# eigenkernel/eigenkernel

Hardware: AMD Instinct MI355X
Metric: eigenpairs/s (full spectrum) + achieved fp64 TFLOP/s vs roofline, N=16384 GEP (higher is better)
Workload: dtype f64

## Files before the change

### eigenkernel_amd/csrc/ek_chol.hip

```cpp
#include "ek_common.h"
#include "ek_block64.h"

#include <cstdlib>
#include <vector>

namespace ek {
namespace {

constexpr int NB = kDiagNB;
constexpr size_t kDiagLds = 2 * b64::IMG * sizeof(double);

__global__ __launch_bounds__(256) void potrf_diag_kernel(int nb, double *B, int ldb, double *inv, int *info,
                                                         int info_base) {
  using namespace b64;
  extern __shared__ double smem[];
  double *sP = smem, *sQ = smem + IMG;
  __shared__ double s_scr[kScratch];
  const int t = threadIdx.x, lane = t & 63, wave = t >> 6, l15 = lane & 15, l4 = lane >> 4;
  auto upper = [&](int gr, int gc) -> double {
    if (gc < nb) return B[(size_t)gc + (size_t)gr * ldb];
    return (gr == gc) ? 1.0 : 0.0;
  };
  auto fail_exit = [&](int j) {
    if (t == 0) atomicCAS(info, 0, info_base + j + 1);
// ... 198 lines not shown
  static bool attr_set = false;
  if (attr_set) return;
  (void)hipFuncSetAttribute((const void *)potrf_diag_kernel, hipFuncAttributeMaxDynamicSharedMemorySize, kDiagLds);
  (void)hipFuncSetAttribute((const void *)trtri_diag_kernel,
                            hipFuncAttributeMaxDynamicSharedMemorySize, (NB * NB + NB) * sizeof(double));
  attr_set = true;
}

void potrf_lower(hipStream_t s, int n, double *B, int ldb, double *invdiag, int *d_info,
                 double *work) {
  set_attrs();
  if (n <= 0) return;
  potrf_rec(s, n, B, ldb, 0, invdiag, d_info, work);
}

void trtri256_blocks(hipStream_t s, int n, const double *L, int ldl, const double *invdiag, double *inv256, double *scratch) {
  const int nb2 = n / (2 * NB);
  if (nb2 <= 0) return;
  GemmDesc g{};
  g.M = NB; g.N = NB; g.K = NB; g.transA = false; g.transB = false; g.alpha = 1.0; g.beta = 0.0; g.batch = nb2; g.lower_only = false;
  g.A = L + NB; g.lda = ldl; g.strideA = (long long)2 * NB * ((long long)ldl + 1);
  g.B = invdiag; g.ldb = NB; g.strideB = (long long)2 * NB * NB;
  g.C = scratch; g.ldc = NB; g.strideC = (long long)NB * NB;
  gemm(s, g);
  g.alpha = -1.0;
  g.A = invdiag + (size_t)NB * NB; g.lda = NB; g.strideA = (long long)2 * NB * NB;
  g.B = scratch; g.ldb = NB; g.strideB = (long long)NB * NB;
  g.C = inv256 + NB; g.ldc = 2 * NB; g.strideC = (long long)4 * NB * NB;
  gemm(s, g);
  hipLaunchKernelGGL(inv256_assemble_kernel, dim3(nb2), dim3(256), 0, s, invdiag, inv256);
}
void trsm_register_inv256(const double *invdiag, const double *inv256, int n) {
  g_inv256.base128 = inv256 ? invdiag : nullptr; g_inv256.inv256 = inv256; g_inv256.nblk256 = inv256 ? n / (2 * NB) : 0;
// ... 123 lines not shown
int sygst_set_direct(int order) {
  const int before = g_sygst_direct;
  g_sygst_direct = order <= 0 ? kSygstDirect : (order < 2 * NB ? 2 * NB : order);
  return before;
}
void sygst_scratch_need(int n, size_t need[2]) {
  if (n <= sygst_direct()) return;
  const size_t n1 = (size_t)split_t(n), n2 = (size_t)n - n1;
  const size_t t1 = n1 * n1 + n1 * n2, t2 = (n1 > n2 ? n1 : n2) * (size_t)n;
  if (t1 > need[0]) need[0] = t1;
  if (t2 > need[1]) need[1] = t2;
  sygst_scratch_need((int)n1, need);
  sygst_scratch_need((int)n2, need);
}

static void sygst_rec(hipStream_t s, int n, double *A, int lda, const double *L, int ldl,
                      const double *invdiag, double *work, double *scratch) {
  if (n <= 0) return;
  if (n <= sygst_direct()) {
    symmetrize_lower(s, n, A, lda);
    trsm_lln(s, n, n, L, ldl, invdiag, A, lda, work);
    trsm_rlt_lower(s, n, L, ldl, invdiag, A, lda, work);
    return;
  }
  const int n1 = split_t(n), n2 = n - n1;
  double *A21 = A + n1, *A22 = A + (size_t)n1 + (size_t)n1 * lda;
  const double *L21 = L + n1, *L22 = L + (size_t)n1 + (size_t)n1 * ldl;
  const double *inv2 = invdiag + (size_t)(n1 / NB) * NB * NB;
  sygst_rec(s, n1, A, lda, L, ldl, invdiag, work, scratch);
  trsm_rlt(s, n2, n1, L, ldl, invdiag, A21, lda, work);
  double *C11 = scratch, *M = scratch + (size_t)n1 * n1;
  hipLaunchKernelGGL(full_from_lower_kernel, grid_mn(n1, n1), dim3(256), 0, s, n1, A, lda, C11, n1);
  gemm(s, false, false, n2, n1, n1, 1.0, L21, ldl, C11, n1, 0.0, M, n2);
  hipLaunchKernelGGL(axpy_matrix_kernel, grid_mn(n2, n1), dim3(256), 0, s, n2, n1, -0.5, M, n2, A21, lda);
  if (n2 <= n1) {
    double *P = C11;
    gemm(s, false, true, n2, n2, n1, 1.0, A21, lda, L21, ldl, 0.0, P, n2);
    hipLaunchKernelGGL(syr2k_fold_kernel, dim3(ceil_div(n2, 32), ceil_div(n2, 32)), dim3(256), 0, s, n2, P, n2, A22, lda);
  } else {
    gemm(s, false, true, n2, n2, n1, -1.0, A21, lda, L21, ldl, 1.0, A22, lda, true);
    gemm(s, false, true, n2, n2, n1, -1.0, L21, ldl, A21, lda, 1.0, A22, lda, true);
  }
  hipLaunchKernelGGL(axpy_matrix_kernel, grid_mn(n2, n1), dim3(256), 0, s, n2, n1, -0.5, M, n2, A21, lda);
  trsm_lln(s, n2, n1, L22, ldl, inv2, A21, lda, work);
  sygst_rec(s, n2, A22, lda, L22, ldl, inv2, work, scratch);
}

void sygst_lower(hipStream_t s, int n, double *A, int lda, const double *L, int ldl,
                 const double *invdiag, double *work, double *scratch) {
  if (n <= 0) return;
  sygst_rec(s, n, A, lda, L, ldl, invdiag, work, scratch);
}


__global__ __launch_bounds__(256) void trmm_diag_kernel(int n, int ldd, const double *__restrict__ L, int ldl,
                                                        double *__restrict__ diag) {
  const int b = blockIdx.x, off = b * ldd;
  const int nb = n - off < ldd ? n - off : ldd;
  double *D = diag + (size_t)b * ldd * ldd;
  const int per = ldd * ldd / gridDim.y;
  for (int idx = blockIdx.y * per + threadIdx.x; idx < (blockIdx.y + 1) * per; idx += 256) {
    const int i = idx % ldd, j = idx / ldd;
    D[idx] = (i >= j && i < nb) ? L[(size_t)(off + i) + (size_t)(off + j) * ldl] : 0.0;
  }
}
int trmm_block_ld(int n) { return n > kDiagNB ? 2 * NB : NB; }
// ... 288 lines not shown
      if (e0) { g_pprof.mark(s); g_pprof.kind.push_back(1); }
      if (has_next) issue_strip(s, k + 1, cur ^ 1);
      waited = true;
    }
  }
  for (int m = 0; m < nmem; ++m)
    hipLaunchKernelGGL(info_to_double_kernel, dim3(ceil_div(NRB, 256)), dim3(256), 0, s, NRB, infos[m], infod[m]);
  x.allreduce(s, nmem, infod, (size_t)NRB, x.user);
  for (int m = 0; m < nmem; ++m)
    hipLaunchKernelGGL(first_info_kernel, dim3(1), dim3(64), 0, s, NRB, infod[m], mem[m].d_info);
}

size_t potrf_rl_work_bytes(int n, int ld) { return PotrfDistLayout(n, ld, 1).total; }

void potrf_lower_rl(hipStream_t s, hipStream_t s2, int n, double *B, int ldb, double *invdiag, int *d_info,
                    void *work) {
  set_attrs();
  if (n <= 0) return;
  const PotrfDistLayout Ly(n, ldb, 1);
  const int NRB = Ly.NRB;
  char *w = (char *)work;
  double *ppan = (double *)(w + Ly.off_pbuf);
  int *infos = (int *)(w + Ly.off_infos);
  double *infod = (double *)(w + Ly.off_infod);
  long long *offs = (long long *)(w + Ly.off_offs);
  int *dims = (int *)(w + Ly.off_dims);
  static hipEvent_t evU[2], evP[2], evFork;
  static bool ev_ready = false;
  if (!ev_ready) {
    for (int i = 0; i < 2; ++i) {
      (void)hipEventCreateWithFlags(&evU[i], hipEventDisableTiming);
      (void)hipEventCreateWithFlags(&evP[i], hipEventDisableTiming);
    }
    (void)hipEventCreateWithFlags(&evFork, hipEventDisableTiming);
    ev_ready = true;
  }
  (void)hipMemsetAsync(infos, 0, (size_t)NRB * sizeof(int), s);
  hipLaunchKernelGGL(potrf_table_kernel, dim3(NRB), dim3(round_up(Ly.maxb, 64)), 0, s, n, ldb, 1, 0, NRB, Ly.maxb,
                     offs, dims);
  auto factor_panel = [&](hipStream_t st, int k) {
    const int off = k * NB, nbk = (n - off < NB) ? n - off : NB, mrows = n - off - nbk;
    double *Bd = B + (size_t)off + (size_t)off * ldb;
    double *inv = invdiag + (size_t)k * NB * NB;
    hipLaunchKernelGGL(potrf_diag_kernel, dim3(1), dim3(256), kDiagLds, st, nbk, Bd,
                       ldb, inv, infos + k, off);
    if (mrows > 0) {
      gemm(st, false, true, mrows, nbk, nbk, 1.0, Bd + nbk, ldb, inv, NB, 0.0, ppan, mrows);
      copy_matrix(st, mrows, nbk, ppan, mrows, Bd + nbk, ldb);
    }
// ... 5 lines not shown
    for (int k = k0; k < k1; ++k) {
      factor_panel(st, k);
      const int cnt = k1 - 1 - k;
      if (cnt > 0) {
        const int nbk = (n - k * NB < NB) ? n - k * NB : NB;
        GemmDesc g{};
        g.N = NB; g.K = nbk; g.transA = false; g.transB = true; g.alpha = -1.0; g.beta = 1.0;
        g.A = B; g.lda = ldb; g.B = B; g.ldb = ldb; g.C = B; g.ldc = ldb; g.lower_only = true;
        g.even_offs = true;
        g.M = n - (k + 1) * NB; g.batch = cnt;
        g.d_offs = offs + (size_t)k * Ly.maxb * 3; g.d_dims = dims + (size_t)k * Ly.maxb * 3;
        gemm(st, g);
      }
    }
  };
  (void)hipEventRecord(evFork, s);
  (void)hipStreamWaitEvent(s2, evFork, 0);
  factor_outer(s2, 0);
  (void)hipEventRecord(evP[0], s2);
  for (int o = 0; o + 1 < NOB; ++o) {
    const int c0 = o * ob * NB, c1 = (o + 1) * ob * NB, kw = c1 - c0;
    const int m2 = n - c1;
    const int wnext = (m2 < ob * NB) ? m2 : ob * NB;
    (void)hipStreamWaitEvent(s, evP[o & 1], 0);
    const double *P = B + (size_t)c1 + (size_t)c0 * ldb;
    double *C = B + (size_t)c1 + (size_t)c1 * ldb;
    gemm(s, false, true, m2, wnext, kw, -1.0, P, ldb, P, ldb, 1.0, C, ldb, true);
    (void)hipEventRecord(evU[(o + 1) & 1], s);
    if (m2 > wnext)
      gemm(s, false, true, m2 - wnext, m2 - wnext, kw, -1.0, P + wnext, ldb, P + wnext, ldb, 1.0,
           C + (size_t)wnext + (size_t)wnext * ldb, ldb, true);
    (void)hipStreamWaitEvent(s2, evU[(o + 1) & 1], 0);
    factor_outer(s2, o + 1);
    (void)hipEventRecord(evP[(o + 1) & 1], s2);
  }
  (void)hipStreamWaitEvent(s, evP[(NOB - 1) & 1], 0);
  hipLaunchKernelGGL(info_to_double_kernel, dim3(ceil_div(NRB, 256)), dim3(256), 0, s, NRB, infos, infod);
  hipLaunchKernelGGL(first_info_kernel, dim3(1), dim3(64), 0, s, NRB, infod, d_info);
}

size_t sygst_dist_scratch_doubles(int n, int ld, int nranks) {
  const int NRB = ceil_div(n > 0 ? n : 1, NB);
  return (size_t)ld * NB * ceil_div(NRB, nranks > 0 ? nranks : 1);
}

void sygst_lower_dist(hipStream_t s, int n, int nmem, const SygstMember *mem, const SytrdExchange &x) {
  if (n <= 0 || nmem <= 0 || nmem > kMaxTeam) return;
  const int P = x.nranks;
  const int NRB = ceil_div(n, NB);
  const int wblk = ceil_div(NRB, P) * NB;
  size_t offs[kMaxTeam], counts[kMaxTeam];
  for (int r = 0; r < P; ++r) {
    long long c0 = (long long)r * wblk, c1 = c0 + wblk;
// ... 34 lines not shown
```

### eigenkernel_amd/csrc/ek_common.h

```cpp
#pragma once
#include <hip/hip_runtime.h>
#include <cstddef>
#include <cstdint>
#include <cstdio>

#define EK_HIP_CHECK(expr)                                                              \
  do {                                                                                  \
    hipError_t _e = (expr);                                                             \
    if (_e != hipSuccess) {                                                             \
      fprintf(stderr, "[ek_hip] %s failed at %s:%d: %s\n", #expr, __FILE__, __LINE__,   \
              hipGetErrorString(_e));                                                   \
      return -1000 - (int)_e;                                                           \
    }                                                                                   \
  } while (0)

namespace ek {

constexpr int kWave = 64;

inline int ceil_div(int a, int b) { return (a + b - 1) / b; }
inline int round_up(int a, int b) { return ceil_div(a, b) * b; }

struct GemmDesc {
  int M, N, K;
// ... 59 lines not shown
constexpr int kDiagNB = 128;
void potrf_lower(hipStream_t s, int n, double *B, int ldb, double *invdiag, int *d_info,
                 double *work );
void trtri_diag_blocks(hipStream_t s, int n, const double *L, int ldl, double *invdiag);
void trsm_rlt(hipStream_t s, int m, int n, const double *L, int ldl, const double *invdiag,
              double *X, int ldx, double *work);
void trsm_lln(hipStream_t s, int n, int m, const double *L, int ldl, const double *invdiag,
              double *X, int ldx, double *work);
void trsm_llt(hipStream_t s, int n, int m, const double *L, int ldl, const double *invdiag,
              double *X, int ldx, double *work);
inline size_t sygst_scratch_doubles(int n) {
  const size_t h = (size_t)(n / 2 + 128);
  const size_t a = 2 * h * h, b = 2 * 128 * 128;
  return a > b ? a : b;
}
void trtri256_blocks(hipStream_t s, int n, const double *L, int ldl, const double *invdiag, double *inv256, double *scratch);
void trsm_register_inv256(const double *invdiag, const double *inv256, int n);
void sygst_lower(hipStream_t s, int n, double *A, int lda, const double *L, int ldl,
                 const double *invdiag, double *work, double *scratch);
int sygst_set_direct(int order);
void sygst_scratch_need(int n, size_t need[2]);
int trmm_block_ld(int n);
size_t trmm_diag_doubles(int n);
void trmm_diag_blocks(hipStream_t s, int n, const double *L, int ldl, double *diag);
void trmm_rln(hipStream_t s, int m, int n, const double *L, int ldl, const double *diag, int ldd,
              double *X, int ldx, double *work);
void trmm_llt(hipStream_t s, int n, int m, const double *L, int ldl, const double *diag, int ldd,
              double *X, int ldx, double *work);
void trmm_lln(hipStream_t s, int n, int m, const double *L, int ldl, const double *diag, int ldd,
              double *X, int ldx, double *work);
void sygst2_lower(hipStream_t s, int n, double *A, int lda, const double *L, int ldl, const double *diag,
                  double *work, double *scratch);
struct SygstMember {
  double *A; int lda; const double *L; int ldl; const double *invdiag;
  double *work;
  double *scratch;
  int rank;
};
size_t potrf_rl_work_bytes(int n, int ld);
void potrf_lower_rl(hipStream_t s, hipStream_t s2, int n, double *B, int ldb, double *invdiag, int *d_info,
                    void *work);
struct SytrdExchange;
struct PotrfMember { double *B; int ldb; double *invdiag; int *d_info; void *work; int rank; };
size_t potrf_dist_work_bytes(int n, int ld, int nranks);
void potrf_lower_dist(hipStream_t s, hipStream_t s2, int n, int nmem, const PotrfMember *mem, const SytrdExchange &x);
void potrf_dist_set_lookahead(int on);
void potrf_dist_profile(bool on);
void potrf_dist_profile_collect(double *seconds, int P);
size_t sygst_dist_scratch_doubles(int n, int ld, int nranks);
void sygst_lower_dist(hipStream_t s, int n, int nmem, const SygstMember *mem, const SytrdExchange &x);

struct SytrdWork;
size_t sytrd_work_bytes(int n);
void sytrd_lower(hipStream_t s, int n, double *A, int lda, double *d, double *e, double *tau,
                 double *V, int ldv, void *work);

// ... 105 lines not shown
```

### eigenkernel_amd/csrc/ek_debug.hip

```cpp
#include "ek_api_internal.h"

using namespace ek;
using namespace ek::api;

extern "C" {

int ek_hip_potrf_team(int n, double *B_loc, const int desc_B[9], int nteam, long long *mismatch) {
  if (n < 0) return -1;
  if (!B_loc && n > 0) return -2;
  int rc = check_desc(desc_B, 3, n, n); if (rc) return rc;
  if (nteam < 0 || nteam > kMaxTeam) return -4;
  rc = ensure_init(); if (rc) return rc;
  if (mismatch) *mismatch = 0;
  if (n == 0) return 0;
  std::lock_guard<std::mutex> lk(g_mu);
  if (nteam == 0 && !g_comm.on) return -4;
  hipStream_t s = g_ctx.stream;
  const int ld = pad_ld(n), nblk = ceil_div(n, kDiagNB);
  const int nmem = nteam > 0 ? nteam : 1, P = nteam > 0 ? nteam : g_comm.nranks;
  const size_t wb = potrf_dist_work_bytes(n, ld, P);
  const size_t per = al((size_t)ld * ld * 8) + al((size_t)nblk * kDiagNB * kDiagNB * 8) + al(wb) + 256;
  void *ws;
  rc = workspace(per * nmem + 256, &ws);
  if (rc) return rc;
// ... 206 lines not shown
  return sy2sb_on_host_arrays(n, A, lda, V, ldv, tau, 0, flag);
}

int ek_hip_debug_sy2sb_stage(int n, double *A, int lda, double *V, int ldv, double *tau, int poison, int *flag) {
  if (n < 1) return -1;
  if (!A) return -2;
  if (lda < n) return -3;
  if (!V) return -4;
  if (ldv < n) return -5;
  if (!tau) return -6;
  if (!flag) return -8;
  return sy2sb_on_host_arrays(n, A, lda, V, ldv, tau, poison, flag);
}

int ek_hip_debug_set_sy2sb_flow(int pair_min, int lookahead_min) { sy2sb_set_flow(pair_min, lookahead_min); return 0; }

__global__ void band_to_matrix_kernel(int n, const double *__restrict__ AB, double *__restrict__ A, int lda) {
  const int c = blockIdx.x;
  for (int d = threadIdx.x; d <= kBandW; d += blockDim.x)
    if (c + d < n) A[(size_t)(c + d) + (size_t)c * lda] = AB[(size_t)d + (size_t)c * kBandLd];
}

int ek_hip_debug_sy2sb_team(int n, double *A, int lda, double *V, int ldv, double *tau, int nteam, int *flag,
                            long long *mismatch) {
  if (n < 1 || !A || !V || !tau || lda < n || ldv < n) return -1;
  if (nteam < 0 || nteam > kMaxTeam) return -7;
  int rc = ensure_init(); if (rc) return rc;
  std::lock_guard<std::mutex> lk(g_mu);
  if (nteam == 0 && !g_comm.on) return -7;
  hipStream_t s = g_ctx.stream;
// ... 705 lines not shown
```

### eigenkernel_amd/csrc/ek_solve.hip

```cpp
#include "ek_api_internal.h"

namespace ek {
namespace api {

void gather_band_strips(hipStream_t s, int n, int nmem, int rank0, double *const *ABs, const SytrdExchange &x) {
  const int NRB = ceil_div(n, 128), P = x.nranks;
  if (P <= 1) return;
  for (int q = 0; q * P < NRB; ++q) {
    size_t offs[kMaxTeam], counts[kMaxTeam];
    for (int r = 0; r < P; ++r) {
      const int S = q * P + r;
      const int cols = (S < NRB) ? ((n - S * 128 < 128) ? n - S * 128 : 128) : 0;
      offs[r] = (S < NRB) ? (size_t)S * 128 * kBandLd : 0; counts[r] = (size_t)cols * kBandLd;
    }
    x.allgatherv(s, nmem, rank0, ABs, offs, counts, P, x.user);
  }
}

}
}

using namespace ek;
using namespace ek::api;

// ... 4 lines not shown
  int made = 0;
  int init() {
    for (auto &e : ev) { EK_HIP_CHECK(hipEventCreate(&e)); ++made; }
    return 0;
  }
  ~StageTimer() { for (int i = 0; i < made; ++i) (void)hipEventDestroy(ev[i]); }
};

int g_debug_fail_chase = 0;
int g_debug_dc_team = 0;

struct PathPlan {
  int ld, nblk, zcols;
  bool two_stage, potrf_rl, compact_dc;
  size_t mat, zmat, x0, x1, sygst_dbl, potrf_wb, wb_sytrd, wb_stedc, wb_ormtr, wb_sy2sb, wb_sb2st, wb_rec, wb_q1prep,
         trsm_work, inv256, total;
};
PathPlan plan_path(int problem, int n, int n_vec, int nc_loc, int nranks_dist ,
                   size_t exch_bytes = 0 ,
                   bool values_only = false, bool value_window = false) {
  PathPlan p{};
  const bool dist = nranks_dist > 0;
  p.ld = pad_ld(n); p.nblk = ceil_div(n, kDiagNB);
  const int ts_min = two_stage_min();
  p.two_stage = ts_min > 0 && n >= ts_min && n >= 3;
  p.mat = al((size_t)p.ld * p.ld * 8);
  p.compact_dc = stedc_compact(n, nc_loc);
  p.zcols = p.compact_dc ? round_up(nc_loc > 0 ? nc_loc : 1, 128) : p.ld;
  p.zmat = al((size_t)p.ld * p.zcols * 8);
  p.wb_sytrd = (p.two_stage) ? 0 : (dist ? sytrd_dist_work_bytes(n, nranks_dist) : sytrd_work_bytes(n));
  p.wb_stedc = stedc_work_bytes(n, nc_loc);
// ... 1 lines not shown
  p.trsm_work = al((size_t)256 * p.ld * 8);
  p.inv256 = (problem == 1) ? al((size_t)(n / 256 > 0 ? n / 256 : 1) * 256 * 256 * 8) : 0;
  p.sygst_dbl = (problem == 1) ? sygst_scratch_doubles(n) : 0;
  if (problem == 1 && dist) {
    const size_t dd = sygst_dist_scratch_doubles(n, p.ld, nranks_dist);
    if (dd > p.sygst_dbl) p.sygst_dbl = dd;
  }
  p.potrf_rl = problem == 1 && n >= kPotrfRlMin;
  p.potrf_wb = (problem == 1 && dist) ? al(potrf_dist_work_bytes(n, p.ld, nranks_dist)) : 0;
  if (p.potrf_rl && al(potrf_rl_work_bytes(n, p.ld)) > p.potrf_wb) p.potrf_wb = al(potrf_rl_work_bytes(n, p.ld));
  p.wb_sy2sb = p.two_stage ? al(dist ? sy2sb_dist_work_bytes(n, nranks_dist) : sy2sb_work_bytes(n)) : 0;
  p.wb_sb2st = p.two_stage ? al(sb2st_work_bytes(n, false)) : 0;
  p.wb_rec = p.two_stage ? al(sb2st_record_bytes(n)) : 0;
  p.wb_q1prep = p.two_stage ? al(ormtr_prep_bytes(n)) : 0;
  p.x0 = p.mat;
  const size_t phase_a = al(p.sygst_dbl * 8) + p.potrf_wb + al(p.wb_sytrd) + 512;
  p.x1 = phase_a;
  if (values_only) {
    p.zcols = 0; p.zmat = 0; p.wb_stedc = 0; p.wb_ormtr = 0; p.wb_rec = 0; p.wb_q1prep = 0;
    if (al(stebz_work_bytes(n)) > p.x1) p.x1 = al(stebz_work_bytes(n));
    if (p.x1 < 4096) p.x1 = 4096;
  }
  if (al(p.wb_stedc) > p.x1) p.x1 = al(p.wb_stedc);
  if (p.wb_rec > p.x1) p.x1 = p.wb_rec;
  if (al(p.wb_ormtr) > p.x1) p.x1 = al(p.wb_ormtr);
  if (al(exch_bytes) > p.x1) p.x1 = al(exch_bytes);
  if (value_window) {
    const size_t dc = al(stedc_work_bytes(n, n - n / 2));
    if (dc > p.x1) p.x1 = dc;
    for (int c = 128; ; c += 128) {
      const int mc = c < n ? c : n;
      if (al(ormtr_work_bytes(n, mc, mc)) > p.x1) p.x1 = al(ormtr_work_bytes(n, mc, mc));
// ... 14 lines not shown
  int nc_out = 0, nr_loc = 0, nc_loc = 0;
  bool dist = false, split_rows = false, values_only = false, value_window = false;
  PathPlan pl{};
  int ld = 0;
  bool two_stage = false, aliasA = false, aliasB = false, aliasZ = false;
  double *wB = nullptr, *wV = nullptr, *wZ = nullptr, *x0 = nullptr, *dInv = nullptr, *twork = nullptr, *dd = nullptr,
         *de = nullptr, *dt = nullptr, *dwv = nullptr, *dt1 = nullptr, *inv256 = nullptr;
  char *x1 = nullptr, *work_sy2sb = nullptr, *work_sb2st = nullptr, *q1prep = nullptr;
  double *wA = nullptr, *wV2 = nullptr;
  double *sscr = nullptr; char *pwork = nullptr; void *sytrd_work = nullptr;
  char *work = nullptr; double *q2rec = nullptr;
  Inv256Guard inv256_guard;
  StageTimer tm;
  bool timing = false;
  int evi = 0;
  void mark() { if (timing) (void)hipEventRecord(tm.ev[evi++], s); }
  double sigma = 1.0;
  bool band_input = false;
  bool two_stage_done = false, window_too_small = false;
  double rescued_panels = 0.0;
  int zslab = 0;
  int stage_in_A(), stage_in_B(), reduce(), tridiagonalise(), chase_with_repeat(), count_window(), values_tail(),
      divide_and_conquer(), stage_out(), finish(bool full), slab_width(int c0) const;
  void cholesky(), a_out(), back_transform(), recover(), z_out(int c0, int nc), exchange_rows();
};

Path::Path(const PathCall &call) : PathCall(call) {
  nc_out = cell ? numroc0(n_vec, cell->nb, cell->mycol, cell->npcol) : n_vec;
  nr_loc = cell ? numroc0(n, cell->nb, cell->myrow, cell->nprow) : n;
  dist = cell && g_comm.on && g_comm.nranks == cell->nprow * cell->npcol;
  if (dist && g_comm.rank != cell->myrow * cell->npcol + cell->mycol) { rc = -994; return; }
  split_rows = dist && cell->nprow > 1;
  nc_loc = split_rows ? numroc0(n_vec, cell->nb, g_comm.rank, g_comm.nranks) : nc_out;
  size_t exch_bytes = 0;
  if (split_rows) exch_bytes = ((size_t)n * (nc_loc > 0 ? nc_loc : 1) + (size_t)(nr_loc > 0 ? nr_loc : 1) * (nc_out > 0 ? nc_out : 1)) * 8 + 4096;
  values_only = win && win->jobz == 0;
// ... 25 lines not shown
  dd = a.get<double>(ld); de = a.get<double>(ld); dt = a.get<double>(ld); dwv = a.get<double>(ld);
  dt1 = a.get<double>(ld);
  work_sy2sb = two_stage ? a.get<char>(pl.wb_sy2sb) : nullptr;
  work_sb2st = two_stage ? a.get<char>(pl.wb_sb2st) : nullptr;
  q1prep = (two_stage && !values_only) ? a.get<char>(pl.wb_q1prep) : nullptr;
  inv256 = pl.inv256 ? (double *)a.get<char>(pl.inv256) : nullptr;
  wA = aliasA ? dA : x0;
  wV2 = x0;
  sscr = (problem == 1) ? (double *)x1 : nullptr;
  pwork = pl.potrf_wb ? x1 + al(pl.sygst_dbl * 8) : nullptr;
  work = x1;
  q2rec = (double *)x1;
  char *sytrd_arena = x1 + al(pl.sygst_dbl * 8) + pl.potrf_wb + 256;
  sytrd_work = two_stage ? nullptr : choose_sytrd_scratch(n, ld, x0, sytrd_arena, dd, pl.wb_sytrd);
  timing = stage_seconds && n_stages > 0;
}

int Path::run() {
  if (rc) return rc;
  if (timing) EK_TRY(tm.init());
  EK_HIP_CHECK(hipMemsetAsync(g_ctx.d_info, 0, 4 * sizeof(int), s));
  mark();
  EK_HIP_CHECK(hipMemsetAsync(wV, 0, (size_t)ld * ld * 8, s));
  EK_HIP_CHECK(hipMemsetAsync(dd, 0, 4 * al((size_t)ld * 8), s));
  if (!pipe) EK_TRY(stage_in_A());
  EK_TRY(stage_in_B());
  mark();
  cholesky();
  mark();
  if (pipe) {
    EK_TRY(stage_in_A());
    if (problem == 1) {
      if (!aliasB) copy_matrix(s, n, n, wB, ld, dB, ldb);
      pipe_out(pipe, s, 'B', dB, ldb, n, 0, n);
    }
  }
  EK_TRY(reduce());
  mark();
  EK_TRY(tridiagonalise());
  mark();
  EK_TRY(count_window());
  if (values_only || (win && (win->m == 0 || window_too_small))) return values_tail();
  EK_TRY(divide_and_conquer());
  mark();
  back_transform();
  mark();
  recover();
  mark();
  EK_TRY(stage_out());
  mark();
  return finish(true);
}

int Path::stage_in_B() {
  if (problem != 1) return 0;
  if (pipe) EK_TRY(pipe_wait_in(pipe, 0));
  if (aliasB) return 0;
  if (ld != n) EK_HIP_CHECK(hipMemsetAsync(wB, 0, (size_t)ld * ld * 8, s));
  copy_matrix(s, n, n, dB, ldb, wB, ld);
  return 0;
}

int Path::stage_in_A() {
  if (pipe) EK_TRY(pipe_wait_in(pipe, 1));
  if (!aliasA) {
    if (ld != n) EK_HIP_CHECK(hipMemsetAsync(wA, 0, (size_t)ld * ld * 8, s));
    copy_matrix(s, n, n, dA, lda, wA, ld);
  }
// ... 2 lines not shown
  double part[512];
  EK_HIP_CHECK(hipMemcpyAsync(part, d_part, sizeof(part), hipMemcpyDeviceToHost, s));
  EK_HIP_CHECK(hipStreamSynchronize(s));
  double anrm = 0.0, offband = 0.0;
  for (int q = 0; q < 256; ++q) { if (part[q] > anrm) anrm = part[q]; if (!(part[256 + q] <= offband)) offband = part[256 + q]; }
  band_input = switch_int(kSwBandInput) != 0 && problem == 0 && !dist && offband == 0.0;
  if (!(anrm <= 1.7e308)) return -4;
  const double rmin = 1e-90, rmax = 1e90;
  if (anrm > 0.0 && anrm < rmin) sigma = rmin / anrm;
  else if (anrm > rmax) sigma = rmax / anrm;
  if (sigma != 1.0) scale_lower(s, n, sigma, wA, ld);
  return 0;
}

void Path::cholesky() {
  if (problem == 1) {
    if (dist && g_comm.nranks >= dist_min_ranks()) {
      const PotrfMember me{wB, ld, dInv, g_ctx.d_info, pwork, g_comm.rank};
      potrf_lower_dist(s, g_ctx.stream2, n, 1, &me, team_exchange(0));
    } else if (pl.potrf_rl) {
      potrf_lower_rl(s, g_ctx.stream2, n, wB, ld, dInv, g_ctx.d_info, pwork);
    } else {
      potrf_lower(s, n, wB, ld, dInv, g_ctx.d_info, twork);
    }
  }
  if (problem == 1 && n >= 256 && (itype == 1 || (itype == 2 && !values_only))) {
    trtri256_blocks(s, n, wB, ld, dInv, inv256, twork);
    trsm_register_inv256(dInv, inv256, n);
  }
}

int Path::reduce() {
  if (problem != 1) return 0;
  if (dist && g_comm.nranks >= dist_min_ranks()) {
    const SygstMember me{wA, ld, wB, ld, dInv, twork, sscr, g_comm.rank};
    sygst_lower_dist(s, n, 1, &me, team_exchange(0));
  } else if (itype == 1) {
    sygst_lower(s, n, wA, ld, wB, ld, dInv, twork, sscr);
  } else {
    trmm_diag_blocks(s, n, wB, ld, wV);
    sygst2_lower(s, n, wA, ld, wB, ld, wV, twork, sscr);
    EK_HIP_CHECK(hipMemsetAsync(wV, 0, trmm_diag_doubles(n) * 8, s));
  }
  return 0;
}

void Path::a_out() {
  if (!aliasA) copy_matrix(s, n, n, wA, ld, dA, lda);
  if (pipe) pipe_out(pipe, s, 'A', dA, lda, n, 0, n);
}

int Path::tridiagonalise() {
  if (dist && !two_stage) {
// ... 209 lines not shown
      if (bad < 0) {
        if (g_comm.err) fprintf(stderr, "[ek_hip] exchange failed: %s\n", comm_error_string());
        return -996;
      }
    }
    if (bad) return -992;
  }
  if (info[0] != 0) return info[0];
  if (full && info[1] != 0) return 100000 + info[1];
  return 0;
}

}

extern "C" {

int ek_hip_solve_device(int problem, int n, int n_vec, double *dA, int lda, double *dB, int ldb,
                        double *dw, double *dZ, int ldz, double *stage_seconds, int n_stages) {
  int rc = solve_args(problem, n, n_vec, dA, lda, dB, ldb, dw, dZ); if (rc) return rc;
  if (ldz < (n > 1 ? n : 1)) return -10;
  rc = ensure_init(); if (rc) return rc;
  if (n == 0) return 0;
  std::lock_guard<std::mutex> lk(g_mu);
  return solve_device_locked(path_call(problem, n, n_vec, dA, lda, dB, ldb, dw, dZ, ldz, stage_seconds, n_stages));
}

int ek_hip_eigenvalues_device(int problem, int n, int il, int iu, double *dA, int lda, double *dB, int ldb,
                              double *dw, double *stage_seconds, int n_stages) {
  int rc = eigenvalues_args(problem, n, il, iu, dA, lda, dB, ldb, dw); if (rc) return rc;
  rc = ensure_init(); if (rc) return rc;
// ... 194 lines not shown
```

### eigenkernel_amd/solver.py

```python
import ctypes
import os
from dataclasses import dataclass, field

import numpy as np

from . import descriptor as _d

_HERE = os.path.dirname(os.path.abspath(__file__))
LIB_PATH = os.environ.get("EK_HIP_LIB") or os.path.join(_HERE, "csrc", "libek_hip.so")

N_STAGES = 8
SOLVERS = ("hip", "hip_select", "general_hip", "general_hip_select")
REPLACES = {"hip": "scalapack", "hip_select": "scalapack_select",
            "general_hip": "general_scalapack", "general_hip_select": "general_scalapack_select"}


class LibraryMissing(RuntimeError):
    pass


_lib = None
_dp = ctypes.POINTER(ctypes.c_double)
_ip = ctypes.POINTER(ctypes.c_int)
_llp = ctypes.POINTER(ctypes.c_longlong)
# ... 174 lines not shown
        "ek_hip_eigenpairs_xvbatched_device": (c_int, [c_int, c_int, c_int, _ip, vp, _ip, vp, _ip, vp, vp, _ip, _ip,
                                                       _dp]),
        "ek_hip_eigenpairs_xvbatched": (c_int, [c_int, c_int, c_int, _ip, vp, _ip, vp, _ip, vp, vp, _ip, _ip, _dp]),
        "ek_hip_sygv_xvbatched_device": (c_int, [c_int, c_int, c_int, _ip, vp, _ip, vp, _ip, vp, vp, _ip, _ip, _dp]),
        "ek_hip_sygv_xvbatched": (c_int, [c_int, c_int, c_int, _ip, vp, _ip, vp, _ip, vp, vp, _ip, _ip, _dp]),
        "ek_hip_debug_xvbatched_last": (c_int, [_dp, _ip]),
        "ek_hip_check_xvbatched_device": (c_int, [c_int, c_int, _ip, vp, _ip, vp, _ip, vp, vp, _ip, _ip, _dp, vp, _dp]),
        "ek_hip_check_xvbatched": (c_int, [c_int, c_int, _ip, vp, _ip, vp, _ip, vp, vp, _ip, _ip, _dp, vp, _dp]),
        "ek_hip_check_sygv_xvbatched_device": (c_int, [c_int, c_int, _ip, vp, _ip, vp, _ip, vp, vp, _ip, _ip, _dp, vp,
                                                       _dp]),
        "ek_hip_check_sygv_xvbatched": (c_int, [c_int, c_int, _ip, vp, _ip, vp, _ip, vp, vp, _ip, _ip, _dp, vp, _dp]),
        "ek_hip_debug_check_xvbatched_last": (c_int, [_dp, _ip]),
        "ek_hip_debug_stage_leaves256": (c_int, [c_int]),
        "ek_hip_debug_set_sygst_direct": (c_int, [c_int]),
        "ek_hip_debug_sygst_scratch": (c_ull, [c_int, ctypes.POINTER(c_ull)]),
        "ek_hip_solve_sparse": (c_int, [c_int, c_int, c_int, c_ll, _ip, _dp, c_ll, _ip, _dp, _dp, _dp, _ip,
                                        c_int, c_int, c_int, c_int, _dp, c_int]),
        "ek_hip_check_sparse_device": (c_int, [c_int, c_int, c_ll, _ip, _dp, c_ll, _ip, _dp, vp, vp, c_int,
                                               c_int, c_int, c_int, c_int, _dp, _dp]),
        "ek_hip_check_sparse": (c_int, [c_int, c_int, c_ll, _ip, _dp, c_ll, _ip, _dp, _dp, _dp, c_int,
                                        c_int, c_int, c_int, c_int, _dp, _dp]),
        "ek_hip_sparse_to_dense": (c_int, [c_int, c_ll, _ip, _dp, _dp, c_int]),
        "ek_hip_debug_sparse_check_workspace_bytes": (c_ull, [c_int, c_int, c_ll, c_ll, c_int, c_int, c_int, c_int]),
        "ek_hip_debug_sparse_csr": (c_ll, [c_int, c_ll, _ip, _dp, _llp, _ip, _dp]),
    }
    for name, (res, args) in sigs.items():
        try:
            fn = getattr(lib, name)
        except AttributeError:
            if os.environ.get("EK_HIP_BRINGUP") == "1":
# ... 33 lines not shown
    "ek_hip_eigenpairs_vbatched_device", "ek_hip_eigenpairs_vbatched",
    "ek_hip_debug_vbatched_streams", "ek_hip_debug_vbatched_last",
    "ek_hip_check_batched_device", "ek_hip_check_batched", "ek_hip_check_vbatched_device", "ek_hip_check_vbatched",
    "ek_hip_sygv_batched_device", "ek_hip_sygv_batched", "ek_hip_sygv_vbatched_device", "ek_hip_sygv_vbatched",
    "ek_hip_check_sygv_batched_device", "ek_hip_check_sygv_batched", "ek_hip_check_sygv_vbatched_device",
    "ek_hip_check_sygv_vbatched", "ek_hip_check_sygvx_device", "ek_hip_check_sygvx",
    "ek_hip_eigenpairs_xbatched_device", "ek_hip_eigenpairs_xbatched", "ek_hip_debug_xbatched_chunk",
    "ek_hip_check_xbatched_device", "ek_hip_check_xbatched", "ek_hip_debug_check_xbatched_chunk",
    "ek_hip_sygv_xbatched_device", "ek_hip_sygv_xbatched",
    "ek_hip_check_sygv_xbatched_device", "ek_hip_check_sygv_xbatched",
    "ek_hip_eigenpairs_xvbatched_device", "ek_hip_eigenpairs_xvbatched", "ek_hip_sygv_xvbatched_device",
    "ek_hip_sygv_xvbatched", "ek_hip_debug_xvbatched_last",
    "ek_hip_check_xvbatched_device", "ek_hip_check_xvbatched", "ek_hip_check_sygv_xvbatched_device",
    "ek_hip_check_sygv_xvbatched", "ek_hip_debug_check_xvbatched_last",
    "ek_hip_debug_stage_leaves256", "ek_hip_debug_set_sygst_direct", "ek_hip_debug_sygst_scratch",
    "ek_hip_solve_sparse", "ek_hip_check_sparse_device", "ek_hip_check_sparse", "ek_hip_sparse_to_dense",
    "ek_hip_debug_sparse_check_workspace_bytes", "ek_hip_debug_sparse_csr",
    "ek_hip_eigenpairs_window_batched_device", "ek_hip_eigenpairs_window_batched", "ek_hip_debug_window_batched_chunk",
)


def _check(what, A, B, w, Z, n_cols, index1=1, index2=1):
    lib = load_library()
    Z = _farr(Z)
    n = Z.shape[0]
    A_ = _farr(A) if A is not None else None
    B_ = _farr(B) if B is not None else None
    out = np.zeros(max(3, n))
    wv = np.ascontiguousarray(np.asarray(w, dtype=np.float64)) if w is not None else np.zeros(max(n, 1))
    info = lib.ek_hip_check(what, 1 if B is not None else 0, n, n_cols, index1, index2,
# ... 321 lines not shown

def trmm(L, Z):
    lib = load_library()
    L = _farr(L)
    Z = np.array(_farr(Z), order="F", copy=True)
    info = lib.ek_hip_trmm(L.shape[0], Z.shape[1], _P(L), _I(_desc_for(L)), _P(Z), _I(_desc_for(Z)))
    return Z, info


def stage_leaves256(mode):
    return int(load_library().ek_hip_debug_stage_leaves256(int(mode)))


def set_sygst_direct(order=0):
    return int(load_library().ek_hip_debug_set_sygst_direct(int(order)))


def sygst_scratch(n):
    need = (ctypes.c_ulonglong * 2)(0, 0)
    have = load_library().ek_hip_debug_sygst_scratch(int(n), need)
    return int(have), int(need[0]), int(need[1])


BAND_W = 64


def set_two_stage(min_order=-1):
    load_library().ek_hip_debug_set_two_stage(int(min_order))


# ... 732 lines not shown
```

### include/ek_hip_debug.h

```cpp
#ifndef EK_HIP_DEBUG_H
#define EK_HIP_DEBUG_H

#ifdef __cplusplus
extern "C" {
#endif

int ek_hip_profile_symv(int enable);
int ek_hip_profile_symv_get(double *seconds, long long *launches, double *algorithmic_bytes);

int ek_hip_profile_kernels(int enable);
int ek_hip_profile_kernels_get(double *seconds , long long *launches );

int ek_hip_debug_sytrd(int n, int ld, int reps, double *seconds);
unsigned long long ek_hip_debug_sytrd_work_bytes(int n);
int ek_hip_debug_sytrd_at(int n, int max_cols, int reps, double *dA, void *work, double *vecs, double *seconds);
int ek_hip_debug_gemm_at(int transa, int transb, int m, int n, int k, const double *dA, int lda, const double *dB,
                         int ldb, double beta, double *dC, int ldc, int lower_only, int reps, double *seconds);
int ek_hip_debug_gemm_desc(int transa, int transb, int m, int n, int k, double alpha, double beta, const double *dA, int lda,
                           long long strideA, const double *dB, int ldb, long long strideB, double *dC, int ldc,
                           long long strideC, int batch, int lower_only, int staged_rank_k, int small_tiles, int even_offs,
                           const long long *offs, const int *dims, int *variant );
int ek_hip_debug_gemm_plan(int transa, int transb, int m, int n, int k, double alpha, double beta, const double *dA, int lda,
                           long long strideA, const double *dB, int ldb, long long strideB, double *dC, int ldc,
                           long long strideC, int batch, int lower_only, int staged_rank_k, int small_tiles, int even_offs,
// ... 28 lines not shown
unsigned long long ek_hip_debug_sparse_check_workspace_bytes(int problem, int n, long long nnzA, long long nnzB,
                                                             int n_check, int index1, int index2, int n_ipr);
long long ek_hip_debug_sparse_csr(int n, long long nnz, const int *suf, const double *val, long long *rowptr, int *col,
                                  double *csr_val);
int ek_hip_debug_vbatched_streams(int streams);
int ek_hip_debug_vbatched_last(double *class_seconds, int *class_count);
int ek_hip_debug_xvbatched_last(double *class_seconds, int *class_count);
int ek_hip_debug_xbatched_chunk(int problems);
int ek_hip_debug_window_batched_chunk(int problems);
int ek_hip_debug_check_xbatched_chunk(int problems);
int ek_hip_debug_check_xvbatched_last(double class_seconds[4], int class_count[4]);

int ek_hip_debug_stage_leaves256(int mode);
int ek_hip_debug_set_sygst_direct(int order);
unsigned long long ek_hip_debug_sygst_scratch(int n, unsigned long long *need );

int ek_hip_debug_fail_next_chase(int times);

int ek_hip_debug_stedc_team(int nranks, int levels, int profile);
int ek_hip_debug_stedc_team_get(double *seconds);

int ek_hip_debug_stedc(int n, const double *d, const double *e, int nsel, int first, int nb, int npcol, int mycol,
                       double *w, double *Z, int ldz, int *merges, int merge_cap, int *info);
int ek_hip_debug_stedc_zcols(int n, int nsel);

int ek_hip_debug_ormtr(int n, int ncols, const double *V, int ldv, const double *tau, double *Z, int ldz,
                       int ncols_global, int slab);

int ek_hip_debug_potrf_team_profile(int lookahead, int profile);
int ek_hip_debug_potrf_team_profile_get(int nteam, double *parts);
// ... 8 lines not shown
```

Measured before the change: 20570.

## Overlap Cholesky tail with sygst front and fork sygst TRSMs to side stream

Splits the right-looking Cholesky so that once enough columns exist for sygst's first recursive block, the remaining trailing updates, panel factors and inv256 block inversions move to the second stream. Meanwhile the main stream starts the sygst recursion, waiting on a tail event only where the rest of L is needed. Inside sygst, the off-diagonal TRSMs are forked to the side stream alongside the recursive diagonal subproblem. This is meant to hide serial Cholesky-tail and TRSM latency behind concurrent GEMM work. The cost is extra event synchronisation, a second workspace and the risk of the two streams competing for compute units.

```diff
diff --git a/eigenkernel_amd/csrc/ek_chol.hip b/eigenkernel_amd/csrc/ek_chol.hip
--- a/eigenkernel_amd/csrc/ek_chol.hip
+++ b/eigenkernel_amd/csrc/ek_chol.hip
@@ -236,9 +236,12 @@
   potrf_rec(s, n, B, ldb, 0, invdiag, d_info, work);
 }
 
-void trtri256_blocks(hipStream_t s, int n, const double *L, int ldl, const double *invdiag, double *inv256, double *scratch) {
-  const int nb2 = n / (2 * NB);
-  if (nb2 <= 0) return;
+void trtri256_blocks(hipStream_t s, int n, const double *L, int ldl, const double *invdiag, double *inv256, double *scratch,
+                     int b0, int b1) {
+  if (b1 < 0 || b1 > n / (2 * NB)) b1 = n / (2 * NB);
+  const int nb2 = b1 - b0;
+  if (b0 < 0 || nb2 <= 0) return;
+  L += (size_t)b0 * 2 * NB * ((size_t)ldl + 1); invdiag += (size_t)b0 * 2 * NB * NB; inv256 += (size_t)b0 * 4 * NB * NB;
   GemmDesc g{};
   g.M = NB; g.N = NB; g.K = NB; g.transA = false; g.transB = false; g.alpha = 1.0; g.beta = 0.0; g.batch = nb2; g.lower_only = false;
   g.A = L + NB; g.lda = ldl; g.strideA = (long long)2 * NB * ((long long)ldl + 1);
@@ -392,10 +395,31 @@
   sygst_scratch_need((int)n2, need);
 }
 
+namespace {
+struct SygstRun {
+  hipStream_t s2 = nullptr; double *work2 = nullptr; hipEvent_t tail = nullptr;
+  bool forks = false;
+  bool live = false;
+};
+hipEvent_t fork_event() {
+  static hipEvent_t ring[16];
+  static int made = 0, next = 0;
+  if (!made) { for (auto &e : ring) (void)hipEventCreateWithFlags(&e, hipEventDisableTiming); made = 1; }
+  next = (next + 1) & 15;
+  return ring[next];
+}
+inline void stream_after(hipStream_t to, hipStream_t from) {
+  hipEvent_t e = fork_event();
+  (void)hipEventRecord(e, from);
+  (void)hipStreamWaitEvent(to, e, 0);
+}
+}
+
 static void sygst_rec(hipStream_t s, int n, double *A, int lda, const double *L, int ldl,
-                      const double *invdiag, double *work, double *scratch) {
+                      const double *invdiag, double *work, double *scratch, SygstRun &run, bool top) {
   if (n <= 0) return;
   if (n <= sygst_direct()) {
+    if (top && run.tail) (void)hipStreamWaitEvent(s, run.tail, 0);
     symmetrize_lower(s, n, A, lda);
     trsm_lln(s, n, n, L, ldl, invdiag, A, lda, work);
     trsm_rlt_lower(s, n, L, ldl, invdiag, A, lda, work);
@@ -405,8 +429,14 @@
   double *A21 = A + n1, *A22 = A + (size_t)n1 + (size_t)n1 * lda;
   const double *L21 = L + n1, *L22 = L + (size_t)n1 + (size_t)n1 * ldl;
   const double *inv2 = invdiag + (size_t)(n1 / NB) * NB * NB;
-  sygst_rec(s, n1, A, lda, L, ldl, invdiag, work, scratch);
-  trsm_rlt(s, n2, n1, L, ldl, invdiag, A21, lda, work);
+  const bool fork1 = run.live;
+  if (fork1) {
+    stream_after(run.s2, s);
+    trsm_rlt(run.s2, n2, n1, L, ldl, invdiag, A21, lda, run.work2);
+  }
+  sygst_rec(s, n1, A, lda, L, ldl, invdiag, work, scratch, run, false);
+  if (fork1) stream_after(s, run.s2);
+  else trsm_rlt(s, n2, n1, L, ldl, invdiag, A21, lda, work);
   double *C11 = scratch, *M = scratch + (size_t)n1 * n1;
   hipLaunchKernelGGL(full_from_lower_kernel, grid_mn(n1, n1), dim3(256), 0, s, n1, A, lda, C11, n1);
   gemm(s, false, false, n2, n1, n1, 1.0, L21, ldl, C11, n1, 0.0, M, n2);
@@ -420,14 +450,43 @@
     gemm(s, false, true, n2, n2, n1, -1.0, L21, ldl, A21, lda, 1.0, A22, lda, true);
   }
   hipLaunchKernelGGL(axpy_matrix_kernel, grid_mn(n2, n1), dim3(256), 0, s, n2, n1, -0.5, M, n2, A21, lda);
-  trsm_lln(s, n2, n1, L22, ldl, inv2, A21, lda, work);
-  sygst_rec(s, n2, A22, lda, L22, ldl, inv2, work, scratch);
+  if (top) {
+    if (run.tail) (void)hipStreamWaitEvent(s, run.tail, 0);
+    run.live = run.forks;
+  }
+  const bool fork2 = run.live;
+  if (fork2) {
+    stream_after(run.s2, s);
+    trsm_lln(run.s2, n2, n1, L22, ldl, inv2, A21, lda, run.work2);
+  } else {
+    trsm_lln(s, n2, n1, L22, ldl, inv2, A21, lda, work);
+  }
+  sygst_rec(s, n2, A22, lda, L22, ldl, inv2, work, scratch, run, false);
+  if (fork2) stream_after(s, run.s2);
 }
 
 void sygst_lower(hipStream_t s, int n, double *A, int lda, const double *L, int ldl,
-                 const double *invdiag, double *work, double *scratch) {
-  if (n <= 0) return;
-  sygst_rec(s, n, A, lda, L, ldl, invdiag, work, scratch);
+                 const double *invdiag, double *work, double *scratch, const SygstSide *side) {
+  SygstRun run;
+  if (side && side->s2) {
+    run.s2 = side->s2; run.work2 = side->work2; run.tail = side->tail;
+    run.forks = side->forks && side->work2;
+    run.live = run.forks && !run.tail;
+  }
+  if (n <= 0) {
+    if (run.tail) (void)hipStreamWaitEvent(s, run.tail, 0);
+    return;
+  }
+  sygst_rec(s, n, A, lda, L, ldl, invdiag, work, scratch, run, true);
+}
+int sygst_first_split(int n) { return n > sygst_direct() ? split_t(n) : 0; }
+
+static int g_overlap_mask = kOverlapAll;
+int overlap_mask() { return g_overlap_mask; }
+int overlap_set_mask(int mask) {
+  const int before = g_overlap_mask;
+  g_overlap_mask = mask & kOverlapAll;
+  return before;
 }
 
 
@@ -746,8 +805,9 @@
 size_t potrf_rl_work_bytes(int n, int ld) { return PotrfDistLayout(n, ld, 1).total; }
 
 void potrf_lower_rl(hipStream_t s, hipStream_t s2, int n, double *B, int ldb, double *invdiag, int *d_info,
-                    void *work) {
+                    void *work, PotrfSplit *split) {
   set_attrs();
+  if (split) split->cstar = 0;
   if (n <= 0) return;
   const PotrfDistLayout Ly(n, ldb, 1);
   const int NRB = Ly.NRB;
@@ -757,7 +817,7 @@
   double *infod = (double *)(w + Ly.off_infod);
   long long *offs = (long long *)(w + Ly.off_offs);
   int *dims = (int *)(w + Ly.off_dims);
-  static hipEvent_t evU[2], evP[2], evFork;
+  static hipEvent_t evU[2], evP[2], evFork, evRest, evReady;
   static bool ev_ready = false;
   if (!ev_ready) {
     for (int i = 0; i < 2; ++i) {
@@ -765,6 +825,8 @@
       (void)hipEventCreateWithFlags(&evP[i], hipEventDisableTiming);
     }
     (void)hipEventCreateWithFlags(&evFork, hipEventDisableTiming);
+    (void)hipEventCreateWithFlags(&evRest, hipEventDisableTiming);
+    (void)hipEventCreateWithFlags(&evReady, hipEventDisableTiming);
     ev_ready = true;
   }
   (void)hipMemsetAsync(infos, 0, (size_t)NRB * sizeof(int), s);
@@ -800,29 +862,41 @@
       }
     }
   };
+  int osplit = -1;
+  if (split && split->ready_cols > 0 && ceil_div(split->ready_cols, ob * NB) < NOB) osplit = ceil_div(split->ready_cols, ob * NB) - 1;
   (void)hipEventRecord(evFork, s);
   (void)hipStreamWaitEvent(s2, evFork, 0);
   factor_outer(s2, 0);
   (void)hipEventRecord(evP[0], s2);
+  hipStream_t su = s;
   for (int o = 0; o + 1 < NOB; ++o) {
     const int c0 = o * ob * NB, c1 = (o + 1) * ob * NB, kw = c1 - c0;
     const int m2 = n - c1;
     const int wnext = (m2 < ob * NB) ? m2 : ob * NB;
-    (void)hipStreamWaitEvent(s, evP[o & 1], 0);
+    if (o == osplit) {
+      (void)hipEventRecord(evReady, s2);
+      (void)hipEventRecord(evRest, s);
+      (void)hipStreamWaitEvent(s2, evRest, 0);
+      (void)hipStreamWaitEvent(s, evReady, 0);
+      su = s2;
+      split->cstar = c1;
+    } else if (su == s) {
+      (void)hipStreamWaitEvent(s, evP[o & 1], 0);
+    }
     const double *P = B + (size_t)c1 + (size_t)c0 * ldb;
     double *C = B + (size_t)c1 + (size_t)c1 * ldb;
-    gemm(s, false, true, m2, wnext, kw, -1.0, P, ldb, P, ldb, 1.0, C, ldb, true);
-    (void)hipEventRecord(evU[(o + 1) & 1], s);
+    gemm(su, false, true, m2, wnext, kw, -1.0, P, ldb, P, ldb, 1.0, C, ldb, true);
+    if (su == s) (void)hipEventRecord(evU[(o + 1) & 1], s);
     if (m2 > wnext)
-      gemm(s, false, true, m2 - wnext, m2 - wnext, kw, -1.0, P + wnext, ldb, P + wnext, ldb, 1.0,
+      gemm(su, false, true, m2 - wnext, m2 - wnext, kw, -1.0, P + wnext, ldb, P + wnext, ldb, 1.0,
            C + (size_t)wnext + (size_t)wnext * ldb, ldb, true);
-    (void)hipStreamWaitEvent(s2, evU[(o + 1) & 1], 0);
+    if (su == s) (void)hipStreamWaitEvent(s2, evU[(o + 1) & 1], 0);
     factor_outer(s2, o + 1);
-    (void)hipEventRecord(evP[(o + 1) & 1], s2);
-  }
-  (void)hipStreamWaitEvent(s, evP[(NOB - 1) & 1], 0);
-  hipLaunchKernelGGL(info_to_double_kernel, dim3(ceil_div(NRB, 256)), dim3(256), 0, s, NRB, infos, infod);
-  hipLaunchKernelGGL(first_info_kernel, dim3(1), dim3(64), 0, s, NRB, infod, d_info);
+    if (su == s) (void)hipEventRecord(evP[(o + 1) & 1], s2);
+  }
+  if (su == s) (void)hipStreamWaitEvent(s, evP[(NOB - 1) & 1], 0);
+  hipLaunchKernelGGL(info_to_double_kernel, dim3(ceil_div(NRB, 256)), dim3(256), 0, su, NRB, infos, infod);
+  hipLaunchKernelGGL(first_info_kernel, dim3(1), dim3(64), 0, su, NRB, infod, d_info);
 }
 
 size_t sygst_dist_scratch_doubles(int n, int ld, int nranks) {
diff --git a/eigenkernel_amd/csrc/ek_common.h b/eigenkernel_amd/csrc/ek_common.h
--- a/eigenkernel_amd/csrc/ek_common.h
+++ b/eigenkernel_amd/csrc/ek_common.h
@@ -97,10 +97,18 @@
   const size_t a = 2 * h * h, b = 2 * 128 * 128;
   return a > b ? a : b;
 }
-void trtri256_blocks(hipStream_t s, int n, const double *L, int ldl, const double *invdiag, double *inv256, double *scratch);
+void trtri256_blocks(hipStream_t s, int n, const double *L, int ldl, const double *invdiag, double *inv256, double *scratch,
+                     int b0 = 0, int b1 = -1);
 void trsm_register_inv256(const double *invdiag, const double *inv256, int n);
+constexpr int kOverlapTail = 1;
+constexpr int kOverlapForks = 2;
+constexpr int kOverlapAll = kOverlapTail | kOverlapForks;
+int overlap_mask();
+int overlap_set_mask(int mask);
+struct SygstSide { hipStream_t s2 = nullptr; double *work2 = nullptr; hipEvent_t tail = nullptr; bool forks = false; };
 void sygst_lower(hipStream_t s, int n, double *A, int lda, const double *L, int ldl,
-                 const double *invdiag, double *work, double *scratch);
+                 const double *invdiag, double *work, double *scratch, const SygstSide *side = nullptr);
+int sygst_first_split(int n);
 int sygst_set_direct(int order);
 void sygst_scratch_need(int n, size_t need[2]);
 int trmm_block_ld(int n);
@@ -121,8 +129,9 @@
   int rank;
 };
 size_t potrf_rl_work_bytes(int n, int ld);
+struct PotrfSplit { int ready_cols = 0; int cstar = 0; };
 void potrf_lower_rl(hipStream_t s, hipStream_t s2, int n, double *B, int ldb, double *invdiag, int *d_info,
-                    void *work);
+                    void *work, PotrfSplit *split = nullptr);
 struct SytrdExchange;
 struct PotrfMember { double *B; int ldb; double *invdiag; int *d_info; void *work; int rank; };
 size_t potrf_dist_work_bytes(int n, int ld, int nranks);
diff --git a/eigenkernel_amd/csrc/ek_debug.hip b/eigenkernel_amd/csrc/ek_debug.hip
--- a/eigenkernel_amd/csrc/ek_debug.hip
+++ b/eigenkernel_amd/csrc/ek_debug.hip
@@ -244,6 +244,11 @@
 }
 
 int ek_hip_debug_set_sy2sb_flow(int pair_min, int lookahead_min) { sy2sb_set_flow(pair_min, lookahead_min); return 0; }
+
+int ek_hip_debug_set_overlap(int mask) {
+  std::lock_guard<std::mutex> lk(g_mu);
+  return overlap_set_mask(mask);
+}
 
 __global__ void band_to_matrix_kernel(int n, const double *__restrict__ AB, double *__restrict__ A, int lda) {
   const int c = blockIdx.x;
diff --git a/eigenkernel_amd/csrc/ek_solve.hip b/eigenkernel_amd/csrc/ek_solve.hip
--- a/eigenkernel_amd/csrc/ek_solve.hip
+++ b/eigenkernel_amd/csrc/ek_solve.hip
@@ -42,7 +42,7 @@
   int ld, nblk, zcols;
   bool two_stage, potrf_rl, compact_dc;
   size_t mat, zmat, x0, x1, sygst_dbl, potrf_wb, wb_sytrd, wb_stedc, wb_ormtr, wb_sy2sb, wb_sb2st, wb_rec, wb_q1prep,
-         trsm_work, inv256, total;
+         trsm_work, inv256, phase_a, total;
 };
 PathPlan plan_path(int problem, int n, int n_vec, int nc_loc, int nranks_dist ,
                    size_t exch_bytes = 0 ,
@@ -74,8 +74,8 @@
   p.wb_rec = p.two_stage ? al(sb2st_record_bytes(n)) : 0;
   p.wb_q1prep = p.two_stage ? al(ormtr_prep_bytes(n)) : 0;
   p.x0 = p.mat;
-  const size_t phase_a = al(p.sygst_dbl * 8) + p.potrf_wb + al(p.wb_sytrd) + 512;
-  p.x1 = phase_a;
+  p.phase_a = al(p.sygst_dbl * 8) + p.potrf_wb + al(p.wb_sytrd) + 512;
+  p.x1 = p.phase_a;
   if (values_only) {
     p.zcols = 0; p.zmat = 0; p.wb_stedc = 0; p.wb_ormtr = 0; p.wb_rec = 0; p.wb_q1prep = 0;
     if (al(stebz_work_bytes(n)) > p.x1) p.x1 = al(stebz_work_bytes(n));
@@ -120,12 +120,19 @@
   StageTimer tm;
   bool timing = false;
   int evi = 0;
-  void mark() { if (timing) (void)hipEventRecord(tm.ev[evi++], s); }
+  void mark(hipStream_t st = nullptr) { if (timing) (void)hipEventRecord(tm.ev[evi++], st ? st : s); }
+  int overlap = 0;
+  double *work2 = nullptr;
+  hipEvent_t ev_tail = nullptr;
+  bool tail_open = false;
+  bool side_used = false;
+  void join_side();
   double sigma = 1.0;
   bool band_input = false;
   bool two_stage_done = false, window_too_small = false;
   double rescued_panels = 0.0;
   int zslab = 0;
+  int run_stages(), run_front(double *dL, int ldl, double *dC, int ldc, int *info);
   int stage_in_A(), stage_in_B(), reduce(), tridiagonalise(), chase_with_repeat(), count_window(), values_tail(),
       divide_and_conquer(), stage_out(), finish(bool full), slab_width(int c0) const;
   void cholesky(), a_out(), back_transform(), recover(), z_out(int c0, int nc), exchange_rows();
@@ -181,9 +188,29 @@
   char *sytrd_arena = x1 + al(pl.sygst_dbl * 8) + pl.potrf_wb + 256;
   sytrd_work = two_stage ? nullptr : choose_sytrd_scratch(n, ld, x0, sytrd_arena, dd, pl.wb_sytrd);
   timing = stage_seconds && n_stages > 0;
+  if (problem == 1 && itype == 1 && pl.potrf_rl && !dist && !cell && !pipe && g_ctx.stream2 && n / 256 < 256 &&
+      sygst_first_split(n) > 0 && pl.x1 >= pl.phase_a + al((size_t)256 * ld * 8)) {
+    overlap = overlap_mask();
+    work2 = (double *)(x1 + pl.phase_a);
+  }
 }
 
 int Path::run() {
+  const int r = run_stages();
+  join_side();
+  return r;
+}
+
+void Path::join_side() {
+  if (!side_used) return;
+  static hipEvent_t ev = nullptr;
+  if (!ev && hipEventCreateWithFlags(&ev, hipEventDisableTiming) != hipSuccess) { (void)hipStreamSynchronize(g_ctx.stream2); return; }
+  (void)hipEventRecord(ev, g_ctx.stream2);
+  (void)hipStreamWaitEvent(s, ev, 0);
+  side_used = false;
+}
+
+int Path::run_stages() {
   if (rc) return rc;
   if (timing) EK_TRY(tm.init());
   EK_HIP_CHECK(hipMemsetAsync(g_ctx.d_info, 0, 4 * sizeof(int), s));
@@ -194,7 +221,7 @@
   EK_TRY(stage_in_B());
   mark();
   cholesky();
-  mark();
+  mark(tail_open ? g_ctx.stream2 : s);
   if (pipe) {
     EK_TRY(stage_in_A());
     if (problem == 1) {
@@ -219,6 +246,22 @@
   return finish(true);
 }
 
+int Path::run_front(double *hL, int ldl, double *hC, int ldc, int *info) {
+  if (rc) return rc;
+  EK_HIP_CHECK(hipMemsetAsync(g_ctx.d_info, 0, 4 * sizeof(int), s));
+  EK_HIP_CHECK(hipMemsetAsync(wV, 0, (size_t)ld * ld * 8, s));
+  EK_HIP_CHECK(hipMemsetAsync(dd, 0, 4 * al((size_t)ld * 8), s));
+  EK_TRY(stage_in_A());
+  EK_TRY(stage_in_B());
+  cholesky();
+  EK_TRY(reduce());
+  join_side();
+  EK_HIP_CHECK(hipGetLastError());
+  EK_TRY(d2h_matrix(n, n, wB, ld, hL, ldl, s));
+  EK_TRY(d2h_matrix(n, n, wA, ld, hC, ldc, s));
+  return fetch_info(info);
+}
+
 int Path::stage_in_B() {
   if (problem != 1) return 0;
   if (pipe) EK_TRY(pipe_wait_in(pipe, 0));
@@ -251,19 +294,33 @@
 }
 
 void Path::cholesky() {
+  PotrfSplit split;
   if (problem == 1) {
     if (dist && g_comm.nranks >= dist_min_ranks()) {
       const PotrfMember me{wB, ld, dInv, g_ctx.d_info, pwork, g_comm.rank};
       potrf_lower_dist(s, g_ctx.stream2, n, 1, &me, team_exchange(0));
     } else if (pl.potrf_rl) {
-      potrf_lower_rl(s, g_ctx.stream2, n, wB, ld, dInv, g_ctx.d_info, pwork);
+      split.ready_cols = (overlap & kOverlapTail) ? sygst_first_split(n) : 0;
+      potrf_lower_rl(s, g_ctx.stream2, n, wB, ld, dInv, g_ctx.d_info, pwork, &split);
     } else {
       potrf_lower(s, n, wB, ld, dInv, g_ctx.d_info, twork);
     }
   }
   if (problem == 1 && n >= 256 && (itype == 1 || (itype == 2 && !values_only))) {
-    trtri256_blocks(s, n, wB, ld, dInv, inv256, twork);
+    if (split.cstar > 0) {
+      trtri256_blocks(s, n, wB, ld, dInv, inv256, twork, 0, split.cstar / 256);
+      trtri256_blocks(g_ctx.stream2, n, wB, ld, dInv, inv256, work2, split.cstar / 256, -1);
+    } else {
+      trtri256_blocks(s, n, wB, ld, dInv, inv256, twork);
+    }
     trsm_register_inv256(dInv, inv256, n);
+  }
+  if (split.cstar > 0) {
+    static hipEvent_t ev = nullptr;
+    if (!ev) (void)hipEventCreateWithFlags(&ev, hipEventDisableTiming);
+    (void)hipEventRecord(ev, g_ctx.stream2);
+    ev_tail = ev;
+    tail_open = side_used = true;
   }
 }
 
@@ -273,7 +330,15 @@
     const SygstMember me{wA, ld, wB, ld, dInv, twork, sscr, g_comm.rank};
     sygst_lower_dist(s, n, 1, &me, team_exchange(0));
   } else if (itype == 1) {
-    sygst_lower(s, n, wA, ld, wB, ld, dInv, twork, sscr);
+    SygstSide side;
+    if (overlap) {
+      side.s2 = g_ctx.stream2; side.work2 = work2;
+      side.tail = tail_open ? ev_tail : nullptr;
+      side.forks = (overlap & kOverlapForks) != 0;
+      if (side.forks) side_used = true;
+    }
+    sygst_lower(s, n, wA, ld, wB, ld, dInv, twork, sscr, &side);
+    tail_open = false;
   } else {
     trmm_diag_blocks(s, n, wB, ld, wV);
     sygst2_lower(s, n, wA, ld, wB, ld, wV, twork, sscr);
@@ -513,6 +578,33 @@
 }
 
 extern "C" {
+
+int ek_hip_debug_front(int n, const double *A, int lda, const double *B, int ldb, double *L, int ldl, double *C, int ldc,
+                       int *info) {
+  if (n < 1) return -1;
+  if (!A) return -2;
+  if (lda < n) return -3;
+  if (!B) return -4;
+  if (ldb < n) return -5;
+  if (!L) return -6;
+  if (ldl < n) return -7;
+  if (!C) return -8;
+  if (ldc < n) return -9;
+  if (!info) return -10;
+  int rc = ensure_init(); if (rc) return rc;
+  std::lock_guard<std::mutex> lk(g_mu);
+  DevMem mem;
+  double *dA = nullptr, *dB = nullptr, *dZ = nullptr, *dw = nullptr;
+  EK_TRY(mem.alloc(&dA, (size_t)n * n * 8)); EK_TRY(mem.alloc(&dB, (size_t)n * n * 8));
+  EK_TRY(mem.alloc(&dZ, (size_t)n * n * 8)); EK_TRY(mem.alloc(&dw, (size_t)n * 8));
+  EK_TRY(h2d_matrix(n, n, A, lda, dA, n, g_ctx.stream));
+  EK_TRY(h2d_matrix(n, n, B, ldb, dB, n, g_ctx.stream));
+  Path path(path_call(1, n, n, dA, n, dB, n, dw, dZ, n, nullptr, 0));
+  rc = path.run_front(L, ldl, C, ldc, info);
+  path.join_side();
+  const hipError_t e = hipStreamSynchronize(g_ctx.stream);
+  return rc ? rc : hip_rc(e);
+}
 
 int ek_hip_solve_device(int problem, int n, int n_vec, double *dA, int lda, double *dB, int ldb,
                         double *dw, double *dZ, int ldz, double *stage_seconds, int n_stages) {
diff --git a/eigenkernel_amd/solver.py b/eigenkernel_amd/solver.py
--- a/eigenkernel_amd/solver.py
+++ b/eigenkernel_amd/solver.py
@@ -212,6 +212,8 @@
         "ek_hip_debug_stage_leaves256": (c_int, [c_int]),
         "ek_hip_debug_set_sygst_direct": (c_int, [c_int]),
         "ek_hip_debug_sygst_scratch": (c_ull, [c_int, ctypes.POINTER(c_ull)]),
+        "ek_hip_debug_set_overlap": (c_int, [c_int]),
+        "ek_hip_debug_front": (c_int, [c_int, _dp, c_int, _dp, c_int, _dp, c_int, _dp, c_int, _ip]),
         "ek_hip_solve_sparse": (c_int, [c_int, c_int, c_int, c_ll, _ip, _dp, c_ll, _ip, _dp, _dp, _dp, _ip,
                                         c_int, c_int, c_int, c_int, _dp, c_int]),
         "ek_hip_check_sparse_device": (c_int, [c_int, c_int, c_ll, _ip, _dp, c_ll, _ip, _dp, vp, vp, c_int,
@@ -275,6 +277,7 @@
     "ek_hip_check_xvbatched_device", "ek_hip_check_xvbatched", "ek_hip_check_sygv_xvbatched_device",
     "ek_hip_check_sygv_xvbatched", "ek_hip_debug_check_xvbatched_last",
     "ek_hip_debug_stage_leaves256", "ek_hip_debug_set_sygst_direct", "ek_hip_debug_sygst_scratch",
+    "ek_hip_debug_set_overlap", "ek_hip_debug_front",
     "ek_hip_solve_sparse", "ek_hip_check_sparse_device", "ek_hip_check_sparse", "ek_hip_sparse_to_dense",
     "ek_hip_debug_sparse_check_workspace_bytes", "ek_hip_debug_sparse_csr",
     "ek_hip_eigenpairs_window_batched_device", "ek_hip_eigenpairs_window_batched", "ek_hip_debug_window_batched_chunk",
@@ -626,6 +629,27 @@
 
 def set_sygst_direct(order=0):
     return int(load_library().ek_hip_debug_set_sygst_direct(int(order)))
+
+
+OVERLAP_TAIL, OVERLAP_FORKS = 1, 2
+OVERLAP_ALL = OVERLAP_TAIL | OVERLAP_FORKS
+
+
+def set_overlap(mask=OVERLAP_ALL):
+    return int(load_library().ek_hip_debug_set_overlap(int(mask)))
+
+
+def front(A, B):
+    lib = load_library()
+    A, B = _farr(A), _farr(B)
+    n = A.shape[0]
+    L = np.zeros((n, n), order="F")
+    C = np.zeros((n, n), order="F")
+    info = ctypes.c_int(0)
+    rc = lib.ek_hip_debug_front(n, _P(A), n, _P(B), n, _P(L), n, _P(C), n, ctypes.byref(info))
+    if rc != 0:
+        raise RuntimeError("ek_hip_debug_front failed: %d" % rc)
+    return L, C, int(info.value)
 
 
 def sygst_scratch(n):
diff --git a/include/ek_hip_debug.h b/include/ek_hip_debug.h
--- a/include/ek_hip_debug.h
+++ b/include/ek_hip_debug.h
@@ -66,6 +66,9 @@
 int ek_hip_debug_stage_leaves256(int mode);
 int ek_hip_debug_set_sygst_direct(int order);
 unsigned long long ek_hip_debug_sygst_scratch(int n, unsigned long long *need );
+int ek_hip_debug_set_overlap(int mask);
+int ek_hip_debug_front(int n, const double *A, int lda, const double *B, int ldb, double *L, int ldl, double *C, int ldc,
+                       int *info);
 
 int ek_hip_debug_fail_next_chase(int times);
 
```

New measurement: 20730, median of 6. Within noise of the previous version (+0.8%).
